# lucidrains/glom-pytorch

Hardware: NVIDIA H100
Metric: column-iterations/sec (BxNxLxiters) at dim=512 L=6 224/14 (higher is better)
Workload: dtype bf16

## Files before the change

### glom_pytorch_b200/csrc/tc_bwd_kernels.cu

```cuda
#include "tc_common.cuh"

#include <stdio.h>

namespace glom {

namespace {

constexpr int BN = 256;
constexpr uint32_t A_BYTES = BM * BK * 2;
constexpr uint32_t B_BYTES = BN * BK * 2;
constexpr uint32_t STAGE_BYTES = A_BYTES + B_BYTES;
constexpr int STAGES = 3;
constexpr int CONSUMER_WARPS = 8;
constexpr int THREADS = 32 * (CONSUMER_WARPS + 1);
constexpr uint32_t PATCH_BYTES = 4096;
constexpr size_t SMEM_BYTES = 1024 + (size_t)STAGES * STAGE_BYTES + 4 * (size_t)STG_BYTES + (size_t)CONSUMER_WARPS * PATCH_BYTES +
                              BN * 4 + 256;

template <int TA, int TB>
__device__ __forceinline__ void kblock(float (&acc)[BN / 2], uint32_t a_smem, uint32_t b_smem) {
  const uint64_t ad = TA ? wgmma_desc_sw128(a_smem, 8192, 1024) : wgmma_desc_sw128(a_smem, 16, 1024);
  const uint64_t bd = TB ? wgmma_desc_sw128(b_smem, 8192, 1024) : wgmma_desc_sw128(b_smem, 16, 1024);
#pragma unroll
  for (int k = 0; k < BK / 16; ++k) wgmma_bf16<BN, TA, TB>(acc, ad + (TA ? (2048 >> 4) : 2) * k, bd + (TB ? (2048 >> 4) : 2) * k);
}

enum { BW_PRE = 0, BW_DH = 1, BW_DX = 2, BW_DW = 3, BW_BATCH = 4 };

struct BwdParams {
  int rows, d, L, n, G;
  int m128;
  int num_tiles;
  const float* b1p;
  __nv_bfloat16* pre;
  __nv_bfloat16* h;
  __nv_bfloat16* dpre;
  float *ds, *d_tokens, *d_pos;
  float *d_bu_w1, *d_bu_w2, *d_td_w1, *d_td_w2;
  float *d_bu_b1, *d_td_b1;
  int bN, bK;
  int a_mn, b_mn;
  int a_state, b_state;
  int out_kind;
  float* out;
  int k_split;
  int a_mn2, b_mn2, a_state2, b_state2;
  const int32_t* steps;
  int t;
  float* dx_td;
  float* b1_part;
  int nbands;
};

__device__ __forceinline__ bool rows_frozen(const BwdParams& p, int r0, int nr, int lane) {
  const int r1 = min(r0 + nr, p.rows);
  bool live = false;
  if (r0 < r1)
    for (int b = r0 / p.n + lane; b <= (r1 - 1) / p.n; b += 32) live |= __ldg(p.steps + b) > p.t;
  return !__any_sync(0xffffffffu, live);
}

__device__ __forceinline__ bool problem_frozen(const BwdParams& p, int z) { return __ldg(p.steps + z / p.L) <= p.t; }

struct Tile {
  int g, m_blk, n_blk, num_kb;
  int kind;
};

template <int MODE>
__device__ __forceinline__ Tile decode(const BwdParams& p, int tile) {
// ... 4 lines not shown
  } else if (MODE == BW_DX) {
    const int nn = p.d / BN, nm = (p.rows + 255) / 256;
    t.n_blk = tile % nn; t.m_blk = (tile / nn) % nm; t.g = tile / (nn * nm); t.num_kb = 4 * p.d / BK;
  } else if (MODE == BW_BATCH) {
    const int nm = (p.n + 255) / 256, nn = (p.bN + BN - 1) / BN;
    t.n_blk = tile % nn; t.m_blk = (tile / nn) % nm; t.g = tile / (nn * nm);
    t.num_kb = p.k_split ? 2 * p.k_split : (p.bK + BK - 1) / BK;
  } else {
    const int per_kind = (p.d / 256) * (4 * p.d / BN);
    t.g = tile / (2 * per_kind);
    const int r = tile % (2 * per_kind);
    t.kind = r / per_kind;
    const int q = r % per_kind;
    const int nn = t.kind == 0 ? 4 * p.d / BN : p.d / BN;
    t.n_blk = q % nn; t.m_blk = q / nn;
    t.num_kb = (p.rows + BK - 1) / BK;
  }
  return t;
}

__device__ __forceinline__ void normal_cdf_pdf(float x, float& cdf, float& pdf) {
  const float a = fabsf(x), t = fminf(a, 6.0f);
  float q = 3.290448512416333e-05f;
  q = fmaf(q, t, -0.0007621519616805017f);
  q = fmaf(q, t, 0.008038812316954136f);
  q = fmaf(q, t, -0.05331535264849663f);
  q = fmaf(q, t, -0.45887142419815063f);
  q = fmaf(q, t, -1.1511567831039429f);
  q = fmaf(q, t, -0.9999995827674866f);
  const float tail = ex2_approx(q);
  cdf = x >= 0.f ? 1.0f - tail : tail;
  float hz = 7.497369551856536e-06f;
  hz = fmaf(hz, t, -0.00023059015802573413f);
  hz = fmaf(hz, t, 0.003048981074243784f);
  hz = fmaf(hz, t, -0.023022783920168877f);
  hz = fmaf(hz, t, 0.11135400831699371f);
  hz = fmaf(hz, t, 0.6360868811607361f);
  hz = fmaf(hz, t, 0.7979033589363098f);
  pdf = tail * hz;
}

template <int MODE, bool DET = false>
__global__ void __launch_bounds__(THREADS, 1)
bwd_gemm_kernel(const __grid_constant__ CUtensorMap map_a0,
                const __grid_constant__ CUtensorMap map_a1,
                const __grid_constant__ CUtensorMap map_a2,
                const __grid_constant__ CUtensorMap map_b,
                const __grid_constant__ CUtensorMap map_b1,
                const __grid_constant__ CUtensorMap map_b2,
                const BwdParams p) {
  extern __shared__ uint8_t smem_raw[];
  uint8_t* smem = smem_raw + ((1024u - (smem_u32(smem_raw) & 1023u)) & 1023u);
  float* stg_all = reinterpret_cast<float*>(smem + (size_t)STAGES * STAGE_BYTES);
  uint8_t* patches = reinterpret_cast<uint8_t*>(stg_all) + 4 * STG_BYTES;
  float* bias_s = reinterpret_cast<float*>(patches + (size_t)CONSUMER_WARPS * PATCH_BYTES);
  uint64_t* full_bar = reinterpret_cast<uint64_t*>(bias_s + BN);
  uint64_t* empty_bar = full_bar + STAGES;

  const int warp = threadIdx.x >> 5, lane = threadIdx.x & 31;
  constexpr int W_TMA = CONSUMER_WARPS;
  const int cta_rank = (int)(blockIdx.x & 1);
  const int cluster_id = blockIdx.x >> 1, num_clusters = gridDim.x >> 1;
  const int kbg_n = 4 * p.d / BK;

  if (warp == W_TMA && lane == 0) {
    for (int i = 0; i < STAGES; ++i) { mbar_init(&full_bar[i], 1); mbar_init(&empty_bar[i], CONSUMER_WARPS); }
    fence_barrier_init();
  }
  __syncthreads();
  pdl_launch_dependents();
  pdl_wait();

  if (warp == W_TMA) {
    const uint32_t elected = elect_one();
    {
      int stage = 0; uint32_t phase = 0;
      for (int tile = cluster_id; tile < p.num_tiles; tile += num_clusters) {
        const Tile t = decode<MODE>(p, tile);
        const int l = t.g >> 1;
        if ((MODE == BW_PRE || MODE == BW_DH || MODE == BW_DX) && p.steps &&
            rows_frozen(p, t.m_blk * 256 + cta_rank * BM, BM, lane))
          continue;
        if (MODE == BW_BATCH && p.steps && problem_frozen(p, t.g)) continue;
        if (MODE == BW_DW && p.steps && rows_frozen(p, 0, p.rows, lane)) continue;
        for (int kb = 0; kb < t.num_kb; ++kb) {
          if (MODE == BW_DW && p.steps && rows_frozen(p, kb * BK, BK, lane)) continue;
          mbar_wait(&empty_bar[stage], phase ^ 1);
          if (elected) {
          const uint32_t sa = smem_u32(smem + (size_t)stage * STAGE_BYTES);
          const uint32_t sb = sa + A_BYTES;
          uint64_t* bar = &full_bar[stage];
          mbar_arrive_expect_tx(bar, STAGE_BYTES);
          if (MODE == BW_PRE || MODE == BW_DH) {
            const int a_row = t.m_blk * 256 + (int)cta_rank * BM;
            const int b_row = t.g * 4 * p.d + t.n_blk * BN;
            if (MODE == BW_PRE) {
              const CUtensorMap* amap = (t.g == 0) ? &map_a0 : ((t.g & 1) ? &map_a2 : &map_a1);
              const int a_col = (t.g == 0) ? 0 : ((t.g & 1) ? l * p.d : (l - 1) * p.d);
              tma_load_2d(sa, amap, bar, a_col + kb * BK, a_row);
            } else {
              tma_load_2d(sa, &map_a0, bar, l * p.d + kb * BK, a_row);
            }
            for (int i = 0; i < 2; ++i) tma_load_2d(sb + i * 16384, &map_b, bar, kb * BK, b_row + i * (BN / 2));
          } else if (MODE == BW_DX) {
            const int m128 = t.m_blk * 2 + (int)cta_rank;
            tma_load_2d(sa, &map_a0, bar, 0, ((t.g * p.m128 + m128) * kbg_n + kb) * BM);
            for (int i = 0; i < 2; ++i) tma_load_2d(sb + i * 16384, &map_b, bar, kb * BK, t.g * p.d + t.n_blk * BN + i * (BN / 2));
          } else if (MODE == BW_BATCH) {
            const int z = t.g, bb = z / p.L, lv = z % p.L;
            const bool seg2 = p.k_split && kb >= p.k_split;
            const int kk = seg2 ? kb - p.k_split : kb;
            const CUtensorMap* am = seg2 ? &map_a1 : &map_a0;
            const CUtensorMap* bm = seg2 ? &map_b1 : &map_b;
            const int a_st = seg2 ? p.a_state2 : p.a_state, b_st = seg2 ? p.b_state2 : p.b_state;
            const int a_mn = seg2 ? p.a_mn2 : p.a_mn, b_mn = seg2 ? p.b_mn2 : p.b_mn;
            const int a_off = a_st ? lv * p.d : 0, a_bt = a_st ? bb : z;
            const int b_off = b_st ? lv * p.d : 0, b_bt = b_st ? bb : z;
            const int mrow = t.m_blk * 256 + cta_rank * BM, ncol = t.n_blk * BN;
            if (!a_mn) tma_load_3d(sa, am, bar, a_off + kk * BK, mrow, a_bt);
            else for (int i = 0; i < 2; ++i) tma_load_3d(sa + i * 8192, am, bar, a_off + mrow + i * 64, kk * BK, a_bt);
            if (!b_mn) for (int i = 0; i < 2; ++i) tma_load_3d(sb + i * 16384, bm, bar, b_off + kk * BK, ncol + i * BM, b_bt);
            else for (int i = 0; i < 4; ++i) tma_load_3d(sb + i * 8192, bm, bar, b_off + ncol + i * 64, kk * BK, b_bt);
          } else {
            const int r0 = kb * BK;
            const int blk_row = (t.g * p.m128 + (r0 >> 7)) * kbg_n;
            const int half = (r0 >> 6) & 1;
            const int mcol = t.m_blk * 256 + cta_rank * BM;
            const int ncol = t.n_blk * BN;
            for (int i = 0; i < 4; ++i) {
              if (t.kind == 0) {
                if (i < 2) tma_load_2d(sa + i * 8192, &map_a0, bar, l * p.d + mcol + i * 64, r0);
                tma_load_2d(sb + i * 8192, &map_a2, bar, 0, (blk_row + (ncol >> 6) + i) * BM + half * 64);
              } else {
                if (i < 2) tma_load_2d(sa + i * 8192, &map_a1, bar, 0, (blk_row + (mcol >> 6) + i) * BM + half * 64);
                const CUtensorMap* bmap = (t.g == 0) ? &map_b : ((t.g & 1) ? &map_b2 : &map_b1);
                const int b_col = (t.g == 0) ? 0 : ((t.g & 1) ? l * p.d : (l - 1) * p.d);
                tma_load_2d(sb + i * 8192, bmap, bar, b_col + ncol + i * 64, r0);
              }
            }
          }
          }
          __syncwarp();
          if (++stage == STAGES) { stage = 0; phase ^= 1; }
        }
      }
    }
  } else if (warp < W_TMA) {
    const int wg = warp >> 2, wi = warp & 3;
    const int quad = warp >> 1, x = warp & 1;
    float* stg = stg_all + quad * (STG_BYTES / 4);
    uint8_t* patch = patches + (size_t)warp * PATCH_BYTES;
    const int c = lane & 7, rsub = lane >> 3;
    const int a_mn1 = (MODE == BW_DW) ? 1 : (MODE == BW_BATCH ? p.a_mn : 0);
    const int b_mn1 = (MODE == BW_DW) ? 1 : (MODE == BW_BATCH ? p.b_mn : 0);
    int stage = 0; uint32_t phase = 0;
    float frag[BN / 2];
    for (int tile = cluster_id; tile < p.num_tiles; tile += num_clusters) {
      const Tile t = decode<MODE>(p, tile);
      if ((MODE == BW_PRE || MODE == BW_DH || MODE == BW_DX) && p.steps &&
          rows_frozen(p, t.m_blk * 256 + cta_rank * BM, BM, lane))
        continue;
      if (MODE == BW_BATCH && p.steps && problem_frozen(p, t.g)) continue;
      if (MODE == BW_DW && p.steps && rows_frozen(p, 0, p.rows, lane)) continue;
      if (MODE == BW_PRE) {
        named_bar_sync(5, CONSUMER_WARPS * 32);
        for (int i = threadIdx.x; i < BN; i += CONSUMER_WARPS * 32) bias_s[i] = __ldg(p.b1p + (size_t)t.g * 4 * p.d + t.n_blk * BN + i);
        named_bar_sync(5, CONSUMER_WARPS * 32);
      }
#pragma unroll
      for (int i = 0; i < BN / 2; ++i) frag[i] = 0.f;
      int prev = -1;
      for (int kb = 0; kb < t.num_kb; ++kb) {
        if (MODE == BW_DW && p.steps && rows_frozen(p, kb * BK, BK, lane)) continue;
        mbar_wait(&full_bar[stage], phase);
        const uint32_t sa = smem_u32(smem + (size_t)stage * STAGE_BYTES) + (uint32_t)wg * 8192u;
        const uint32_t sb = smem_u32(smem + (size_t)stage * STAGE_BYTES) + A_BYTES;
        const bool seg2 = MODE == BW_BATCH && p.k_split && kb >= p.k_split;
        const int sel = seg2 ? 2 * p.a_mn2 + p.b_mn2 : 2 * a_mn1 + b_mn1;
        wgmma_fence_regs(frag);
        wgmma_fence();
        if (sel == 0) kblock<0, 0>(frag, sa, sb);
        else if (sel == 1) kblock<0, 1>(frag, sa, sb);
        else if (sel == 2) kblock<1, 0>(frag, sa, sb);
        else kblock<1, 1>(frag, sa, sb);
        wgmma_commit();
        wgmma_wait<1>();
        wgmma_fence_regs(frag);
        if (prev >= 0) { __syncwarp(); if (lane == 0) mbar_arrive(&empty_bar[prev]); }
        prev = stage;
        if (++stage == STAGES) { stage = 0; phase ^= 1; }
      }
      if (MODE == BW_DW && prev < 0) continue;
      wgmma_wait<0>();
      wgmma_fence_regs(frag);
      __syncwarp();
      if (lane == 0) mbar_arrive(&empty_bar[prev]);
      const int row0 = t.m_blk * 256 + cta_rank * BM + quad * 32;
#pragma unroll 1
      for (int part = 0; part < BN / 64; ++part) {
        const int c0 = 32 * x;
        auto blocked_off = [&](int r) -> size_t {
          const int row = row0 + r, col = t.n_blk * BN + part * 64 + c0 + c * 4;
          return ((size_t)((t.g * p.m128 + (row >> 7)) * kbg_n + (col >> 6)) * BM + (row & 127)) * BK + (col & 63);
        };
        uint2 gp_cur[8];
        if (MODE == BW_DH) {
#pragma unroll
          for (int i = 0; i < 8; ++i) {
            const int r = i * 4 + rsub;
            gp_cur[i] = row0 + r < p.rows ? __ldg(reinterpret_cast<const uint2*>(p.pre + blocked_off(r))) : make_uint2(0u, 0u);
          }
        }
        stage_write(frag, stg, part, wi, lane);
        named_bar_sync(1 + quad, 64);
        uint32_t v[32];
        stage_read(stg, x, lane, v);
#pragma unroll
        for (int j = 0; j < 8; ++j)
          *reinterpret_cast<uint4*>(patch + lane * 128 + ((j ^ (lane & 7)) << 4)) =
              make_uint4(v[4 * j], v[4 * j + 1], v[4 * j + 2], v[4 * j + 3]);
        __syncwarp();
        const int col = t.n_blk * BN + part * 64 + c0 + c * 4;
        float colsum[4] = {0.f, 0.f, 0.f, 0.f};
#pragma unroll
        for (int i = 0; i < 8; ++i) {
          const int r = i * 4 + rsub;
          const float4 acc = *reinterpret_cast<const float4*>(patch + r * 128 + ((c ^ (r & 7)) << 4));
          const int row = row0 + r;
          if (MODE == BW_PRE || MODE == BW_DH) {
            if (row < p.rows) {
              const size_t off = blocked_off(r);
              if (MODE == BW_PRE) {
                const float4 b4 = *reinterpret_cast<const float4*>(bias_s + part * 64 + c0 + c * 4);
                const float xv[4] = {acc.x + b4.x, acc.y + b4.y, acc.z + b4.z, acc.w + b4.w};
                float hv[4], gp[4];
#pragma unroll
                for (int e = 0; e < 4; ++e) {
                  float cdf, pdf;
                  normal_cdf_pdf(xv[e], cdf, pdf);
                  hv[e] = xv[e] * cdf;
                  gp[e] = fmaf(xv[e], pdf, cdf);
                }
                *reinterpret_cast<uint2*>(p.h + off) = make_uint2(pack_bf16x2(hv[0], hv[1]), pack_bf16x2(hv[2], hv[3]));
                *reinterpret_cast<uint2*>(p.pre + off) = make_uint2(pack_bf16x2(gp[0], gp[1]), pack_bf16x2(gp[2], gp[3]));
              } else {
                const uint2 pw = gp_cur[i];
                const float q0 = acc.x * __uint_as_float(pw.x << 16), q1 = acc.y * __uint_as_float(pw.x & 0xFFFF0000u);
                const float q2 = acc.z * __uint_as_float(pw.y << 16), q3 = acc.w * __uint_as_float(pw.y & 0xFFFF0000u);
                colsum[0] += q0; colsum[1] += q1; colsum[2] += q2; colsum[3] += q3;
                *reinterpret_cast<uint2*>(p.dpre + off) = make_uint2(pack_bf16x2(q0, q1), pack_bf16x2(q2, q3));
              }
            }
          } else if (MODE == BW_DX) {
            if constexpr (DET) {
              const int lg = t.g >> 1;
              if (row < p.rows && (t.g & 1)) {
                *reinterpret_cast<float4*>(p.dx_td + ((size_t)row * (p.L - 1) + lg) * p.d + col) = acc;
              } else if (row < p.rows) {
                float* dst = t.g == 0 ? p.d_tokens + (size_t)row * p.d + col : p.ds + ((size_t)row * p.L + lg - 1) * p.d + col;
                float4 o = *reinterpret_cast<const float4*>(dst);
                o.x += acc.x; o.y += acc.y; o.z += acc.z; o.w += acc.w;
                *reinterpret_cast<float4*>(dst) = o;
              }
            } else if (row < p.rows) {
              const int lg = t.g >> 1;
              if (t.g == 0) {
                red_add_f32x4(p.d_tokens + (size_t)row * p.d + col, acc);
              } else if (t.g & 1) {
                red_add_f32x4(p.ds + ((size_t)row * p.L + lg + 1) * p.d + col, acc);
                red_add_f32x4(p.d_pos + (size_t)(row % p.n) * p.d + col, acc);
              } else {
                red_add_f32x4(p.ds + ((size_t)row * p.L + lg - 1) * p.d + col, acc);
              }
            }
          } else if (MODE == BW_BATCH) {
            const int z = t.g;
            if (row < p.n && col < p.bN) {
              if (p.out_kind == 0) {
                float* dst = p.out + ((size_t)z * p.n + row) * p.bN + col;
                if ((p.bN & 3) == 0) *reinterpret_cast<float4*>(dst) = acc;
// ... 166 lines not shown
```

### glom_pytorch_b200/csrc/tc_common.cuh

```cuda
#pragma once
#include "engine.h"
#include "ptx.cuh"

#include <stdio.h>

namespace glom {

constexpr int BM = 128;
constexpr int BK = 64;
constexpr uint32_t A_STAGE_BYTES = BM * BK * 2;

constexpr int STG_PITCH = 68;
constexpr uint32_t STG_BYTES = 32 * STG_PITCH * 4;
template <int S, int R>
__device__ __forceinline__ void stage_write_step(const float (&acc)[R], float* stg, int warp_in_wg, int lane) {
  const int r = 16 * (warp_in_wg & 1) + (lane >> 2), c = 2 * (lane & 3);
#pragma unroll
  for (int j = 0; j < 8; ++j) {
#pragma unroll
    for (int h = 0; h < 2; ++h)
      *reinterpret_cast<float2*>(stg + (r + 8 * h) * STG_PITCH + 8 * j + c) =
          make_float2(acc[4 * (8 * S + j) + 2 * h], acc[4 * (8 * S + j) + 2 * h + 1]);
  }
}
template <int R>
__device__ __forceinline__ void stage_write(const float (&acc)[R], float* stg, int s, int warp_in_wg, int lane) {
  static_assert(R % 32 == 0 && R <= 128, "m64 x N fragment, N in {64, 128, 256}");
  if (s == 0) stage_write_step<0>(acc, stg, warp_in_wg, lane);
  if constexpr (R >= 64) { if (s == 1) stage_write_step<1>(acc, stg, warp_in_wg, lane); }
  if constexpr (R >= 128) {
    if (s == 2) stage_write_step<2>(acc, stg, warp_in_wg, lane);
    if (s == 3) stage_write_step<3>(acc, stg, warp_in_wg, lane);
  }
}
__device__ __forceinline__ void stage_read(const float* stg, int x, int lane, uint32_t (&v)[32]) {
  const float4* src = reinterpret_cast<const float4*>(stg + lane * STG_PITCH + 32 * x);
#pragma unroll
  for (int q = 0; q < 8; ++q) {
    const float4 f = src[q];
    v[4 * q] = __float_as_uint(f.x); v[4 * q + 1] = __float_as_uint(f.y);
    v[4 * q + 2] = __float_as_uint(f.z); v[4 * q + 3] = __float_as_uint(f.w);
  }
}

template <int N, int TB>
__device__ __forceinline__ void wgmma_kblock(float (&acc)[N / 2], uint32_t a_smem, uint32_t b_smem) {
  const uint64_t ad = wgmma_desc_sw128(a_smem, 16, 1024);
  const uint64_t bd = TB ? wgmma_desc_sw128(b_smem, 8192, 1024) : wgmma_desc_sw128(b_smem, 16, 1024);
#pragma unroll
  for (int k = 0; k < BK / 16; ++k) wgmma_bf16<N, 0, TB>(acc, ad + 2 * k, bd + (TB ? (2048 >> 4) : 2) * k);
}

__device__ __forceinline__ float row_chunk_sumsq(float a, float b, float c, float d) {
  float q = a * a;
  q = fmaf(b, b, q);
  q = fmaf(c, c, q);
  q = fmaf(d, d, q);
  q += __shfl_xor_sync(0xffffffffu, q, 1);
  q += __shfl_xor_sync(0xffffffffu, q, 2);
  q += __shfl_xor_sync(0xffffffffu, q, 4);
  return q;
}

struct K2Chunk {
  int l, L, d, n, row0;
  int prow0;
  int s_bcast;
  bool remap;
  const float* s32_in; const __nv_bfloat16* c_in; const float* pos;
  float* s32_out; __nv_bfloat16* sb_out; __nv_bfloat16* sp_out;
};
template <bool FULL, bool SETTLE = false>
__device__ __forceinline__ void k2_chunk(const uint32_t (&v)[32], const float4 b4, uint8_t* patch, const K2Chunk& k,
                                         int col, int lane, int rows_left, float (&rowsq)[8], uint32_t live = ~0u,
                                         float* rowdsq = nullptr, bool want_dsq = false) {
#pragma unroll
  for (int c = 0; c < 8; ++c)
    *reinterpret_cast<uint4*>(patch + lane * 128 + ((c ^ (lane & 7)) << 4)) =
        make_uint4(v[4 * c], v[4 * c + 1], v[4 * c + 2], v[4 * c + 3]);
  __syncwarp();
  const int c = lane & 7, rsub = lane >> 3;
  const bool top = (k.l == k.L - 1);
  const bool has_td = (k.l >= 1);
  const int ld = k.L * k.d, ldp = (k.L - 1) * k.d;
  const size_t base = ((size_t)k.row0 * k.L + k.l) * k.d + col + c * 4;
  const size_t pbase = ((size_t)k.row0 * (k.L - 1) + (k.l - 1)) * k.d + col + c * 4;
#pragma unroll
  for (int h = 0; h < 2; ++h) {
    float4 sv[4], pp[4];
    uint2 cw[4];
#pragma unroll
    for (int j = 0; j < 4; ++j) {
      const int r = (h * 4 + j) * 4 + rsub;
      sv[j] = make_float4(0.f, 0.f, 0.f, 0.f); pp[j] = sv[j]; cw[j] = make_uint2(0u, 0u);
      if ((FULL || r < rows_left) && (!SETTLE || ((live >> r) & 1u))) {
        size_t so = base + (unsigned)(r * ld);
        if (!SETTLE && k.remap) {
          int sr = k.prow0 + r;
          if (k.n >= 32) { if (sr >= k.n) sr -= k.n; } else sr %= k.n;
          so = (size_t)k.l * k.d + col + c * 4 + (unsigned)(sr * ld);
        }
        sv[j] = k.s_bcast ? __ldg(reinterpret_cast<const float4*>(k.s32_in + (size_t)k.l * k.d + col + c * 4))
                          : __ldcs(reinterpret_cast<const float4*>(k.s32_in + so));
        cw[j] = __ldcs(reinterpret_cast<const uint2*>(k.c_in + so));
        if (has_td) {
          int pr = k.prow0 + r;
          if (k.n >= 32) { if (pr >= k.n) pr -= k.n; } else pr %= k.n;
          pp[j] = __ldg(reinterpret_cast<const float4*>(k.pos + (size_t)pr * k.d + col + c * 4));
        }
      }
    }
#pragma unroll
    for (int j = 0; j < 4; ++j) {
      const int i = h * 4 + j;
      const int r = i * 4 + rsub;
      const float4 acc = *reinterpret_cast<const float4*>(patch + r * 128 + ((c ^ (r & 7)) << 4));
      float o0 = (sv[j].x + (acc.x + b4.x)) + __uint_as_float(cw[j].x << 16);
      float o1 = (sv[j].y + (acc.y + b4.y)) + __uint_as_float(cw[j].x & 0xFFFF0000u);
      float o2 = (sv[j].z + (acc.z + b4.z)) + __uint_as_float(cw[j].y << 16);
      float o3 = (sv[j].w + (acc.w + b4.w)) + __uint_as_float(cw[j].y & 0xFFFF0000u);
      if (top) { o0 = o0 / 3.0f; o1 = o1 / 3.0f; o2 = o2 / 3.0f; o3 = o3 / 3.0f; }
      else { o0 *= 0.25f; o1 *= 0.25f; o2 *= 0.25f; o3 *= 0.25f; }
      const bool store = (FULL || r < rows_left) && (!SETTLE || ((live >> r) & 1u));
      if constexpr (SETTLE) if (want_dsq) {
        const float e0 = store ? o0 - sv[j].x : 0.f, e1 = store ? o1 - sv[j].y : 0.f;
        const float e2 = store ? o2 - sv[j].z : 0.f, e3 = store ? o3 - sv[j].w : 0.f;
        rowdsq[i] += row_chunk_sumsq(e0, e1, e2, e3);
      }
      if (store) {
        const size_t o = base + (unsigned)(r * ld);
        __stcs(reinterpret_cast<float4*>(k.s32_out + o), make_float4(o0, o1, o2, o3));
        *reinterpret_cast<uint2*>(k.sb_out + o) = make_uint2(pack_bf16x2(o0, o1), pack_bf16x2(o2, o3));
        if (has_td)
          *reinterpret_cast<uint2*>(k.sp_out + pbase + (unsigned)(r * ldp)) =
              make_uint2(pack_bf16x2(o0 + pp[j].x, o1 + pp[j].y), pack_bf16x2(o2 + pp[j].z, o3 + pp[j].w));
      } else {
        o0 = o1 = o2 = o3 = 0.f;
      }
      rowsq[i] += row_chunk_sumsq(o0, o1, o2, o3);
    }
  }
  __syncwarp();
}

static inline int encode_map(Launch& ln, CUtensorMap* m, const void* base, int rank, const uint64_t* dims,
                             const uint64_t* strides_bytes , const uint32_t* box, const char* what) {
  cuuint64_t gd[3]; cuuint64_t gs[2]; cuuint32_t bx[3]; cuuint32_t es[3] = {1, 1, 1};
  for (int i = 0; i < rank; ++i) { gd[i] = dims[i]; bx[i] = box[i]; }
  for (int i = 0; i < rank - 1; ++i) gs[i] = strides_bytes[i];
  const CUresult r = ln.enc(m, CU_TENSOR_MAP_DATA_TYPE_BFLOAT16, (cuuint32_t)rank, const_cast<void*>(base), gd, gs, bx, es,
                         CU_TENSOR_MAP_INTERLEAVE_NONE, CU_TENSOR_MAP_SWIZZLE_128B, CU_TENSOR_MAP_L2_PROMOTION_L2_256B,
                         CU_TENSOR_MAP_FLOAT_OOB_FILL_NONE);
  if (r != CUDA_SUCCESS) return ln.fail(GLOM_B200_ERR_CUDA, "cuTensorMapEncodeTiled(%s) failed with CUresult %d", what, (int)r);
  return 0;
}

static inline int map2d(Launch& ln, CUtensorMap* m, const void* base, uint64_t rows, uint64_t cols, uint32_t box_rows,
                        const char* what) {
  const uint64_t dims[2] = {cols, rows};
  const uint64_t strides[1] = {cols * 2};
  const uint32_t box[2] = {(uint32_t)BK, box_rows};
  return encode_map(ln, m, base, 2, dims, strides, box, what);
}

}
```

### glom_pytorch_b200/csrc/tc_kernels.cu

```cuda
#include "gemm_sched.cuh"
#include "tc_common.cuh"

#include <stdio.h>
#include <stdlib.h>
#include <string.h>

#include <type_traits>

namespace glom {

constexpr int GEMM_CONSUMER_WARPS = 8;
constexpr int GEMM_THREADS = 128 + 32 * GEMM_CONSUMER_WARPS;
constexpr uint32_t GEMM_PRODUCER_REGS = 40;
constexpr uint32_t GEMM_CONSUMER_REGS = 232;

__device__ unsigned long long g_kernel_clk[PROF_KINDS][8];


template <int MODE, int BN>
struct GemmCfg {
  static constexpr int PARTS = (BN == 256) ? 4 : 2;
  static constexpr int PART_COLS = BN / PARTS;
  static constexpr int THREADS = GEMM_THREADS;
  static constexpr uint32_t B_STAGE_BYTES = BN * BK * 2;
  static constexpr uint32_t STAGE_BYTES = A_STAGE_BYTES + B_STAGE_BYTES;
  static_assert(MODE >= 0 && MODE <= 2, "0 = GEMM1+GELU, 1 = GEMM2+combine, 2 = tokeniser");
  static constexpr int STAGES = (BN == 256) ? 3 : (BN == 128) ? 4 : 5;
  static constexpr uint32_t OUT_BOX_BYTES = 64 * BK * 2;
  static constexpr uint32_t PATCH_BYTES = 4096;
  static constexpr size_t EPI_BYTES = (MODE == 0) ? 2 * (BN / 64) * (size_t)OUT_BOX_BYTES
                                                  : 4 * (size_t)STG_BYTES + (size_t)GEMM_CONSUMER_WARPS * PATCH_BYTES + 4 * 32 * 4;
  static constexpr size_t SMEM_BYTES = 1024  + (size_t)STAGES * STAGE_BYTES + EPI_BYTES + 256 ;
  static_assert(SMEM_BYTES <= 232448, "over the 227 KB of shared memory a block may opt in to");
};

__device__ __forceinline__ void tok_chunk(const uint32_t (&v)[32], const float4 b4, uint8_t* patch, float* dst,
                                          size_t pitch, int lane, int rows_left) {
#pragma unroll
  for (int c = 0; c < 8; ++c)
    *reinterpret_cast<uint4*>(patch + lane * 128 + ((c ^ (lane & 7)) << 4)) =
        make_uint4(v[4 * c], v[4 * c + 1], v[4 * c + 2], v[4 * c + 3]);
  __syncwarp();
  const int c = lane & 7, rsub = lane >> 3;
#pragma unroll
  for (int i = 0; i < 8; ++i) {
    const int r = i * 4 + rsub;
    const float4 a = *reinterpret_cast<const float4*>(patch + r * 128 + ((c ^ (r & 7)) << 4));
    if (r < rows_left)
      *reinterpret_cast<float4*>(dst + (size_t)r * pitch + c * 4) = make_float4(a.x + b4.x, a.y + b4.y, a.z + b4.z, a.w + b4.w);
  }
  __syncwarp();
}

template <int MODE>
__device__ __forceinline__ bool settle_skip(const GemmParams& p, const TileInfo& t) {
  if (p.block_frozen[t.m_blk]) return true;
  return MODE == 0 && t.z == 0 && p.block_fresh != nullptr && !p.block_fresh[t.m_blk];
}

template <int MODE, int BN, bool CNT, bool SETTLE = false>
__global__ void __launch_bounds__(GEMM_THREADS, 1)
gemm_kernel(const __grid_constant__ CUtensorMap map_a0,
            const __grid_constant__ CUtensorMap map_a1,
            const __grid_constant__ CUtensorMap map_a2,
            const __grid_constant__ CUtensorMap map_b,
            const __grid_constant__ CUtensorMap map_out,
            const GemmParams p) {
  using Cfg = GemmCfg<MODE, BN>;
  constexpr int STAGES = Cfg::STAGES;
  constexpr bool RED = MODE != 2 && !SETTLE;
  extern __shared__ uint8_t smem_raw[];
  uint8_t* smem = smem_raw + ((1024u - (smem_u32(smem_raw) & 1023u)) & 1023u);
  uint8_t* epi = smem + (size_t)STAGES * Cfg::STAGE_BYTES;
  float* stg_all = reinterpret_cast<float*>(epi);
  uint8_t* patches = epi + 4 * STG_BYTES;
  float* xch = reinterpret_cast<float*>(patches + (size_t)GEMM_CONSUMER_WARPS * Cfg::PATCH_BYTES);
  uint64_t* full_bar = reinterpret_cast<uint64_t*>(epi + Cfg::EPI_BYTES);
  uint64_t* empty_bar = full_bar + STAGES;

  const int warp = threadIdx.x >> 5;
  const int lane = threadIdx.x & 31;
  constexpr int W_TMA = 0;
  constexpr int W_CONSUMER0 = 4;
  const int cta_rank = (int)(blockIdx.x & 1);
  const int cluster_id = blockIdx.x >> 1;
  const int num_clusters = gridDim.x >> 1;

  if (warp == W_TMA && lane == 0) {
    tma_prefetch_desc(&map_a0);
    tma_prefetch_desc(&map_b);
    if (MODE == 0) { tma_prefetch_desc(&map_a1); tma_prefetch_desc(&map_a2); tma_prefetch_desc(&map_out); }
    for (int i = 0; i < STAGES; ++i) { mbar_init(&full_bar[i], 1); mbar_init(&empty_bar[i], 2 * GEMM_CONSUMER_WARPS); }
    fence_barrier_init();
  }
  cluster_sync_all();
  pdl_launch_dependents();
  pdl_wait();
  const bool clk_thread = blockIdx.x == 0 && warp == W_TMA && lane == 0;
  ClockSample* clk_s = reinterpret_cast<ClockSample*>(empty_bar + STAGES);
  if (clk_thread) *clk_s = clock_sample_begin();
  const bool cnt_cta = CNT && blockIdx.x == 0;
  unsigned long long* const cnt = g_kernel_clk[MODE == 0 ? PROF_GEMM1 : MODE == 1 ? PROF_GEMM2 : PROF_TOKENIZE];
  unsigned long long w0 = 0, w1 = 0;
#define GLOM_CNT_WAIT(acc, stmt) do { if (cnt_cta) { const long long t_ = clock64(); stmt; acc += (unsigned long long)(clock64() - t_); } else { stmt; } } while (0)

  if (warp < W_CONSUMER0) {
    setmaxnreg_dec<GEMM_PRODUCER_REGS>();
    if (warp == W_TMA) {
      const uint32_t elected = elect_one();
      int stage = 0; uint32_t phase = 0;
      const uint32_t smem0 = smem_u32(smem);
      const uint64_t pol_first = l2_policy_evict_first();
      const int kbg_n = 4 * p.d / BK;
      const int blk_skip = (p.m128 - 1) * kbg_n;
      for (int it = 0, tile; (tile = sched_tile<MODE>(p, cluster_id, num_clusters, it)) >= 0; ++it) {
        const TileInfo t = decode_tile<MODE, RED>(p, tile);
        if constexpr (SETTLE) { if (settle_skip<MODE>(p, t)) continue; }
        const CUtensorMap* amap;
        int a_col, b_row;
        if (MODE == 0) {
          const int l = t.z >> 1;
          if (t.z == 0) { amap = &map_a0; a_col = 0; }
          else if (t.z & 1) { amap = &map_a2; a_col = l * p.d; }
          else { amap = &map_a1; a_col = (l - 1) * p.d; }
          b_row = t.z * 4 * p.d + t.n_blk * BN;
        } else if (MODE == 1) {
          amap = &map_a0; a_col = 0;
          b_row = t.z * p.d + t.n_blk * BN;
        } else {
          amap = &map_a0; a_col = 0;
          b_row = t.n_blk * BN;
        }
        const int a_row = t.m_blk * 256 + cta_rank * BM;
        const int blk0 = (2 * t.z * p.m128 + (a_row >> 7)) * kbg_n;
        int td_skip = blk_skip;
        if constexpr (RED && MODE == 1) {
          if (p.num_m_rep > 0 && t.z + 1 >= p.remap_l) td_skip -= ((a_row >> 7) - (a_row >> 7) % p.h_period) * kbg_n;
        }
        for (int kb = 0; kb < t.num_kb; ++kb) {
          GLOM_CNT_WAIT(w0, mbar_wait(&empty_bar[stage], phase ^ 1));
          if (elected) {
            const uint32_t sa = smem0 + (uint32_t)stage * Cfg::STAGE_BYTES;
            uint64_t* bar = &full_bar[stage];
            mbar_arrive_expect_tx(bar, Cfg::STAGE_BYTES);
            if (MODE == 1) {
              const int blk = blk0 + kb + (kb >= kbg_n ? td_skip : 0);
              tma_load_2d_hint(sa, amap, bar, 0, blk * BM, pol_first);
            } else {
              tma_load_2d(sa, amap, bar, a_col + kb * BK, a_row);
            }
            const uint32_t b_half = (uint32_t)cta_rank * (BN / 2);
            tma_load_2d_multicast(sa + A_STAGE_BYTES + b_half * BK * 2, &map_b, bar, kb * BK, b_row + (int)b_half, 0x3);
          }
          __syncwarp();
          if (++stage == STAGES) { stage = 0; phase ^= 1; }
        }
      }
      if (cnt_cta && elected) atomicAdd(&cnt[4], w0);
    }
  } else {
    setmaxnreg_inc<GEMM_CONSUMER_REGS>();
    const int cw = warp - W_CONSUMER0;
    const int wg = cw >> 2, wi = cw & 3;
    const int pair = cw >> 1, x = cw & 1;
    float* stg = stg_all + pair * (STG_BYTES / 4);
    uint8_t* patch = patches + (size_t)cw * Cfg::PATCH_BYTES;
    float* xch_p = xch + pair * 32;
    const uint32_t smem0 = smem_u32(smem);
    const uint64_t pol_stream = l2_policy_evict_first();
    const bool st_issuer = (threadIdx.x & 127) == 0;
    const uint32_t out_wg = smem_u32(epi) + (uint32_t)wg * (BN / 64) * Cfg::OUT_BOX_BYTES;
    const uint32_t st_row = (uint32_t)(16 * wi + 8 * ((lane >> 3) & 1) + (lane & 7)) * 128;
    const int st_jx = lane >> 4, st_sw = lane & 7;
    const uint32_t empty_peer = mapa_shared(smem_u32(empty_bar), (uint32_t)cta_rank ^ 1u);
    auto release = [&](int slot) {
      __syncwarp();
      if (lane == 0) { mbar_arrive(&empty_bar[slot]); mbar_arrive_cluster(empty_peer + 8u * (uint32_t)slot); }
    };
    int stage = 0; uint32_t phase = 0;
    float acc[BN / 2];
    for (int it = 0, tile; (tile = sched_tile<MODE>(p, cluster_id, num_clusters, it)) >= 0; ++it) {
      const TileInfo t = decode_tile<MODE, RED>(p, tile);
      if constexpr (SETTLE) { if (settle_skip<MODE>(p, t)) continue; }
      const int row0 = t.m_blk * 256 + cta_rank * BM + pair * 32;
      const int rows_left = p.rows - row0;
      uint32_t live = ~0u;
      if constexpr (SETTLE && MODE == 1)
        live = __ballot_sync(0xffffffffu, row0 + lane < p.rows && !p.frozen[(row0 + lane) / p.n]);
      bool remap = false;
      if constexpr (RED && MODE == 1) remap = p.num_m_rep > 0 && t.z >= p.remap_l;
      if (MODE == 1 && lane < rows_left) {
        const int src_row = remap ? (row0 + lane) % p.n : row0 + lane;
        const size_t o = ((size_t)src_row * p.L + t.z) * p.d + t.n_blk * BN + x * (BN / 2);
#pragma unroll
        for (int c = 0; c < BN / 2; c += 32) {
          if (!p.s_bcast) prefetch_l2(p.s32_in + o + c);
          if ((c & 63) == 0) prefetch_l2(p.c_in + o + c);
        }
      }
#pragma unroll
      for (int i = 0; i < BN / 2; ++i) acc[i] = 0.f;
      int prev = -1;
      for (int kb = 0; kb < t.num_kb; ++kb) {
        GLOM_CNT_WAIT(w0, mbar_wait(&full_bar[stage], phase));
        const uint32_t sa = smem0 + (uint32_t)stage * Cfg::STAGE_BYTES;
        wgmma_fence_regs(acc);
        wgmma_fence();
        wgmma_kblock<BN, 0>(acc, sa + (uint32_t)wg * (A_STAGE_BYTES / 2), sa + A_STAGE_BYTES);
        wgmma_commit();
        wgmma_wait<1>();
        wgmma_fence_regs(acc);
        if (prev >= 0) release(prev);
        prev = stage;
        if (++stage == STAGES) { stage = 0; phase ^= 1; }
      }
      wgmma_wait<0>();
      wgmma_fence_regs(acc);
      release(prev);
      const long long busy_t0 = cnt_cta ? clock64() : 0;
      if constexpr (MODE == 0) {
        const int wrow0 = t.m_blk * 256 + cta_rank * BM + 64 * wg;
        if (wrow0 < p.rows) {
          const int hblk0 = (t.z * p.m128 + (t.m_blk * 2 + cta_rank)) * (4 * p.d / BK) + t.n_blk * (BN / BK);
          const float* bias = p.bias + (size_t)t.z * 4 * p.d + t.n_blk * BN + 2 * (lane & 3);
          uint32_t pk[BN / 4];
#pragma unroll
          for (int s = 0; s < BN / 64; ++s) {
#pragma unroll
            for (int j = 0; j < 8; ++j) {
              const float2 b = __ldg(reinterpret_cast<const float2*>(bias + 64 * s + 8 * j));
#pragma unroll
              for (int h = 0; h < 2; ++h)
                pk[16 * s + 2 * j + h] = gelu_pair_bf16(acc[4 * (8 * s + j) + 2 * h], acc[4 * (8 * s + j) + 2 * h + 1], b.x, b.y);
            }
          }
          if (st_issuer) bulk_wait_group_read<0>();
          named_bar_sync(1 + wg, 128);
#pragma unroll
          for (int s = 0; s < BN / 64; ++s)
#pragma unroll
            for (int q = 0; q < 4; ++q)
              stmatrix_x4(out_wg + (uint32_t)s * Cfg::OUT_BOX_BYTES + st_row + ((uint32_t)((2 * q + st_jx) ^ st_sw) << 4),
                          pk[16 * s + 4 * q], pk[16 * s + 4 * q + 1], pk[16 * s + 4 * q + 2], pk[16 * s + 4 * q + 3]);
          fence_proxy_async_smem();
          named_bar_sync(1 + wg, 128);
          if (st_issuer) {
#pragma unroll
            for (int s = 0; s < BN / 64; ++s)
              tma_store_2d_hint(&map_out, out_wg + (uint32_t)s * Cfg::OUT_BOX_BYTES, 0, (hblk0 + s) * BM + 64 * wg, pol_stream);
            bulk_commit_group();
          }
        }
      } else {
#pragma unroll 1
        for (int s = 0; s < BN / 64; ++s) {
          stage_write(acc, stg, s, wi, lane);
          named_bar_sync(1 + pair, 64);
          uint32_t v[32];
          stage_read(stg, x, lane, v);
          const int cc = 64 * s + 32 * x;
          if (MODE == 2) {
            float* trow = p.tok_out + (size_t)row0 * p.d + t.n_blk * BN + cc;
            const float4 b4 = __ldg(reinterpret_cast<const float4*>(p.bias + t.n_blk * BN + cc + (lane & 7) * 4));
            tok_chunk(v, b4, patch, trow, (size_t)p.d, lane, rows_left);
          } else {
            K2Chunk kc;
            kc.l = t.z; kc.L = p.L; kc.d = p.d; kc.n = p.n; kc.row0 = row0; kc.prow0 = row0 % p.n; kc.s_bcast = p.s_bcast;
            kc.remap = remap;
            kc.s32_in = p.s32_in; kc.c_in = p.c_in; kc.pos = p.pos;
            kc.s32_out = p.s32_out; kc.sb_out = p.sb_out; kc.sp_out = p.sp_out;
            const int col = t.n_blk * BN + cc;
            const float4 b4 = __ldg(reinterpret_cast<const float4*>(p.bias + (size_t)t.z * p.d + col + (lane & 7) * 4));
            float rowsq[8], rowdsq[8];
#pragma unroll
            for (int i = 0; i < 8; ++i) rowsq[i] = rowdsq[i] = 0.f;
            const bool want_dsq = SETTLE && p.dsq_out != nullptr;
            if (rows_left >= 32) k2_chunk<true, SETTLE>(v, b4, patch, kc, col, lane, 32, rowsq, live, rowdsq, want_dsq);
            else k2_chunk<false, SETTLE>(v, b4, patch, kc, col, lane, rows_left, rowsq, live, rowdsq, want_dsq);
            int part = cc / Cfg::PART_COLS;
            bool writer = true;
            if (Cfg::PART_COLS == 64) {
              float* dxch = reinterpret_cast<float*>(patches + (size_t)(cw | 1) * Cfg::PATCH_BYTES);
              if (x == 1 && (lane & 7) == 0) {
#pragma unroll
                for (int i = 0; i < 8; ++i) xch_p[i * 4 + (lane >> 3)] = rowsq[i];
                if (want_dsq) {
#pragma unroll
                  for (int i = 0; i < 8; ++i) dxch[i * 4 + (lane >> 3)] = rowdsq[i];
                }
              }
              named_bar_sync(1 + pair, 64);
              if (x == 0) {
#pragma unroll
                for (int i = 0; i < 8; ++i) rowsq[i] += xch_p[i * 4 + (lane >> 3)];
                if (want_dsq) {
#pragma unroll
                  for (int i = 0; i < 8; ++i) rowdsq[i] += dxch[i * 4 + (lane >> 3)];
                }
              }
              writer = x == 0;
            }
            if (writer && (lane & 7) == 0) {
              const size_t po = ((size_t)row0 * p.L + t.z) * p.nparts + t.n_blk * Cfg::PARTS + part;
              float* nsq = p.nsq_out + po;
              const int ldn = p.L * p.nparts;
#pragma unroll
              for (int i = 0; i < 8; ++i) {
                const int r = i * 4 + (lane >> 3);
                if (r < rows_left && (!SETTLE || ((live >> r) & 1u))) {
                  nsq[(unsigned)(r * ldn)] = rowsq[i];
                  if (want_dsq) p.dsq_out[po + (unsigned)(r * ldn)] = rowdsq[i];
                }
              }
            }
          }
          named_bar_sync(1 + pair, 64);
        }
      }
      if (cnt_cta) w1 += (unsigned long long)(clock64() - busy_t0);
    }
    if (cnt_cta && cw == 0 && lane == 0) { atomicAdd(&cnt[2], w0); atomicAdd(&cnt[6], w1); }
    if (MODE == 0 && st_issuer) bulk_wait_group<0>();
  }
#undef GLOM_CNT_WAIT

  cluster_sync_all();
  if (clk_thread) clock_sample_end(*clk_s, g_kernel_clk[MODE == 0 ? PROF_GEMM1 : MODE == 1 ? PROF_GEMM2 : PROF_TOKENIZE]);
}

constexpr int ATTN_CONSUMER_WARPS = 8;
constexpr int ATTN_THREADS = 128 + 32 * ATTN_CONSUMER_WARPS;
constexpr uint32_t ATTN_PRODUCER_REGS = 56;
constexpr uint32_t ATTN_CONSUMER_REGS = 224;
constexpr int ATTN_SCALE_WARPS = 3;
constexpr float ATTN_BOUND_MAX = 96.f;
constexpr int ATTN_SINGLE_PASS_MAX = 576;
constexpr int ATTN_PASS_KEYS = 512;

template <int KEYS>
struct AttnCfg {
  static_assert(KEYS == 128 || KEYS == 256, "S block = one wgmma N");
  static constexpr int MAX_KB = (KEYS == 256) ? 1 : 5;
  static constexpr uint32_t SLOT_BYTES = A_STAGE_BYTES + (uint32_t)KEYS * BK * 2;
  static_assert(SLOT_BYTES >= 4 * 8192, "a slot holds a V chunk");
};

struct AttnParams {
  int n, L, d;
  int attend_self, mask_side, mask_d2_max;
  int n_pad16, n_pad64, nkb, nchunk;
// ... 659 lines not shown
```

Before: 67.64 million.

## Read epilogue directly from swizzled staging buffer, drop per-warp patch transpose

The staging buffer now uses an XOR-swizzled 64-float pitch, so epilogue threads can read their row/column float4 straight from it. This removes the extra register round-trip and per-warp patch buffer transpose in the forward and backward epilogues. The freed shared memory goes to deeper TMA pipelines for the non-GELU GEMM modes. k2_chunk also software-pipelines its global loads several rows ahead. The cost is higher register pressure from the prefetch arrays, and the swizzle indexing must match between writer and reader.

```diff
diff --git a/glom_pytorch_b200/csrc/tc_bwd_kernels.cu b/glom_pytorch_b200/csrc/tc_bwd_kernels.cu
--- a/glom_pytorch_b200/csrc/tc_bwd_kernels.cu
+++ b/glom_pytorch_b200/csrc/tc_bwd_kernels.cu
@@ -13,9 +13,7 @@
 constexpr int STAGES = 3;
 constexpr int CONSUMER_WARPS = 8;
 constexpr int THREADS = 32 * (CONSUMER_WARPS + 1);
-constexpr uint32_t PATCH_BYTES = 4096;
-constexpr size_t SMEM_BYTES = 1024 + (size_t)STAGES * STAGE_BYTES + 4 * (size_t)STG_BYTES + (size_t)CONSUMER_WARPS * PATCH_BYTES +
-                              BN * 4 + 256;
+constexpr size_t SMEM_BYTES = 1024 + (size_t)STAGES * STAGE_BYTES + 4 * (size_t)STG_BYTES + BN * 4 + 256;
 
 template <int TA, int TB>
 __device__ __forceinline__ void kblock(float (&acc)[BN / 2], uint32_t a_smem, uint32_t b_smem) {
@@ -126,8 +124,7 @@
   extern __shared__ uint8_t smem_raw[];
   uint8_t* smem = smem_raw + ((1024u - (smem_u32(smem_raw) & 1023u)) & 1023u);
   float* stg_all = reinterpret_cast<float*>(smem + (size_t)STAGES * STAGE_BYTES);
-  uint8_t* patches = reinterpret_cast<uint8_t*>(stg_all) + 4 * STG_BYTES;
-  float* bias_s = reinterpret_cast<float*>(patches + (size_t)CONSUMER_WARPS * PATCH_BYTES);
+  float* bias_s = stg_all + 4 * (STG_BYTES / 4);
   uint64_t* full_bar = reinterpret_cast<uint64_t*>(bias_s + BN);
   uint64_t* empty_bar = full_bar + STAGES;
 
@@ -223,7 +220,6 @@
     const int wg = warp >> 2, wi = warp & 3;
     const int quad = warp >> 1, x = warp & 1;
     float* stg = stg_all + quad * (STG_BYTES / 4);
-    uint8_t* patch = patches + (size_t)warp * PATCH_BYTES;
     const int c = lane & 7, rsub = lane >> 3;
     const int a_mn1 = (MODE == BW_DW) ? 1 : (MODE == BW_BATCH ? p.a_mn : 0);
     const int b_mn1 = (MODE == BW_DW) ? 1 : (MODE == BW_BATCH ? p.b_mn : 0);
@@ -287,19 +283,12 @@
         }
         stage_write(frag, stg, part, wi, lane);
         named_bar_sync(1 + quad, 64);
-        uint32_t v[32];
-        stage_read(stg, x, lane, v);
-#pragma unroll
-        for (int j = 0; j < 8; ++j)
-          *reinterpret_cast<uint4*>(patch + lane * 128 + ((j ^ (lane & 7)) << 4)) =
-              make_uint4(v[4 * j], v[4 * j + 1], v[4 * j + 2], v[4 * j + 3]);
-        __syncwarp();
         const int col = t.n_blk * BN + part * 64 + c0 + c * 4;
         float colsum[4] = {0.f, 0.f, 0.f, 0.f};
 #pragma unroll
         for (int i = 0; i < 8; ++i) {
           const int r = i * 4 + rsub;
-          const float4 acc = *reinterpret_cast<const float4*>(patch + r * 128 + ((c ^ (r & 7)) << 4));
+          const float4 acc = stage_read(stg, x, r, c);
           const int row = row0 + r;
           if (MODE == BW_PRE || MODE == BW_DH) {
             if (row < p.rows) {
diff --git a/glom_pytorch_b200/csrc/tc_common.cuh b/glom_pytorch_b200/csrc/tc_common.cuh
--- a/glom_pytorch_b200/csrc/tc_common.cuh
+++ b/glom_pytorch_b200/csrc/tc_common.cuh
@@ -10,16 +10,18 @@
 constexpr int BK = 64;
 constexpr uint32_t A_STAGE_BYTES = BM * BK * 2;
 
-constexpr int STG_PITCH = 68;
+constexpr int STG_PITCH = 64;
 constexpr uint32_t STG_BYTES = 32 * STG_PITCH * 4;
+__device__ __forceinline__ int stg_swz(int r) { return 2 * (r & 3); }
 template <int S, int R>
 __device__ __forceinline__ void stage_write_step(const float (&acc)[R], float* stg, int warp_in_wg, int lane) {
   const int r = 16 * (warp_in_wg & 1) + (lane >> 2), c = 2 * (lane & 3);
+  const int swz = stg_swz(r);
 #pragma unroll
   for (int j = 0; j < 8; ++j) {
 #pragma unroll
     for (int h = 0; h < 2; ++h)
-      *reinterpret_cast<float2*>(stg + (r + 8 * h) * STG_PITCH + 8 * j + c) =
+      *reinterpret_cast<float2*>(stg + (r + 8 * h) * STG_PITCH + 4 * ((2 * j) ^ swz) + c) =
           make_float2(acc[4 * (8 * S + j) + 2 * h], acc[4 * (8 * S + j) + 2 * h + 1]);
   }
 }
@@ -33,14 +35,8 @@
     if (s == 3) stage_write_step<3>(acc, stg, warp_in_wg, lane);
   }
 }
-__device__ __forceinline__ void stage_read(const float* stg, int x, int lane, uint32_t (&v)[32]) {
-  const float4* src = reinterpret_cast<const float4*>(stg + lane * STG_PITCH + 32 * x);
-#pragma unroll
-  for (int q = 0; q < 8; ++q) {
-    const float4 f = src[q];
-    v[4 * q] = __float_as_uint(f.x); v[4 * q + 1] = __float_as_uint(f.y);
-    v[4 * q + 2] = __float_as_uint(f.z); v[4 * q + 3] = __float_as_uint(f.w);
-  }
+__device__ __forceinline__ float4 stage_read(const float* stg, int x, int r, int c) {
+  return *reinterpret_cast<const float4*>(stg + r * STG_PITCH + 4 * ((8 * x + c) ^ stg_swz(r)));
 }
 
 template <int N, int TB>
@@ -71,76 +67,69 @@
   float* s32_out; __nv_bfloat16* sb_out; __nv_bfloat16* sp_out;
 };
 template <bool FULL, bool SETTLE = false>
-__device__ __forceinline__ void k2_chunk(const uint32_t (&v)[32], const float4 b4, uint8_t* patch, const K2Chunk& k,
-                                         int col, int lane, int rows_left, float (&rowsq)[8], uint32_t live = ~0u,
-                                         float* rowdsq = nullptr, bool want_dsq = false) {
-#pragma unroll
-  for (int c = 0; c < 8; ++c)
-    *reinterpret_cast<uint4*>(patch + lane * 128 + ((c ^ (lane & 7)) << 4)) =
-        make_uint4(v[4 * c], v[4 * c + 1], v[4 * c + 2], v[4 * c + 3]);
-  __syncwarp();
+__device__ __forceinline__ void k2_chunk(const float* stg, int x, const float4 b4, const K2Chunk& k, int col, int lane,
+                                         int rows_left, float (&rowsq)[8], uint32_t live = ~0u, float* rowdsq = nullptr,
+                                         bool want_dsq = false) {
   const int c = lane & 7, rsub = lane >> 3;
   const bool top = (k.l == k.L - 1);
   const bool has_td = (k.l >= 1);
   const int ld = k.L * k.d, ldp = (k.L - 1) * k.d;
   const size_t base = ((size_t)k.row0 * k.L + k.l) * k.d + col + c * 4;
   const size_t pbase = ((size_t)k.row0 * (k.L - 1) + (k.l - 1)) * k.d + col + c * 4;
-#pragma unroll
-  for (int h = 0; h < 2; ++h) {
-    float4 sv[4], pp[4];
-    uint2 cw[4];
-#pragma unroll
-    for (int j = 0; j < 4; ++j) {
-      const int r = (h * 4 + j) * 4 + rsub;
-      sv[j] = make_float4(0.f, 0.f, 0.f, 0.f); pp[j] = sv[j]; cw[j] = make_uint2(0u, 0u);
-      if ((FULL || r < rows_left) && (!SETTLE || ((live >> r) & 1u))) {
-        size_t so = base + (unsigned)(r * ld);
-        if (!SETTLE && k.remap) {
-          int sr = k.prow0 + r;
-          if (k.n >= 32) { if (sr >= k.n) sr -= k.n; } else sr %= k.n;
-          so = (size_t)k.l * k.d + col + c * 4 + (unsigned)(sr * ld);
-        }
-        sv[j] = k.s_bcast ? __ldg(reinterpret_cast<const float4*>(k.s32_in + (size_t)k.l * k.d + col + c * 4))
-                          : __ldcs(reinterpret_cast<const float4*>(k.s32_in + so));
-        cw[j] = __ldcs(reinterpret_cast<const uint2*>(k.c_in + so));
-        if (has_td) {
-          int pr = k.prow0 + r;
-          if (k.n >= 32) { if (pr >= k.n) pr -= k.n; } else pr %= k.n;
-          pp[j] = __ldg(reinterpret_cast<const float4*>(k.pos + (size_t)pr * k.d + col + c * 4));
-        }
+  constexpr int DEPTH = SETTLE ? 4 : 5;
+  float4 sv[8], pp[8];
+  uint2 cw[8];
+  auto load = [&](int i) {
+    const int r = i * 4 + rsub;
+    sv[i] = make_float4(0.f, 0.f, 0.f, 0.f); pp[i] = sv[i]; cw[i] = make_uint2(0u, 0u);
+    if ((FULL || r < rows_left) && (!SETTLE || ((live >> r) & 1u))) {
+      size_t so = base + (unsigned)(r * ld);
+      if (!SETTLE && k.remap) {
+        int sr = k.prow0 + r;
+        if (k.n >= 32) { if (sr >= k.n) sr -= k.n; } else sr %= k.n;
+        so = (size_t)k.l * k.d + col + c * 4 + (unsigned)(sr * ld);
+      }
+      sv[i] = k.s_bcast ? __ldg(reinterpret_cast<const float4*>(k.s32_in + (size_t)k.l * k.d + col + c * 4))
+                        : __ldcs(reinterpret_cast<const float4*>(k.s32_in + so));
+      cw[i] = __ldcs(reinterpret_cast<const uint2*>(k.c_in + so));
+      if (has_td) {
+        int pr = k.prow0 + r;
+        if (k.n >= 32) { if (pr >= k.n) pr -= k.n; } else pr %= k.n;
+        pp[i] = __ldg(reinterpret_cast<const float4*>(k.pos + (size_t)pr * k.d + col + c * 4));
       }
     }
+  };
 #pragma unroll
-    for (int j = 0; j < 4; ++j) {
-      const int i = h * 4 + j;
-      const int r = i * 4 + rsub;
-      const float4 acc = *reinterpret_cast<const float4*>(patch + r * 128 + ((c ^ (r & 7)) << 4));
-      float o0 = (sv[j].x + (acc.x + b4.x)) + __uint_as_float(cw[j].x << 16);
-      float o1 = (sv[j].y + (acc.y + b4.y)) + __uint_as_float(cw[j].x & 0xFFFF0000u);
-      float o2 = (sv[j].z + (acc.z + b4.z)) + __uint_as_float(cw[j].y << 16);
-      float o3 = (sv[j].w + (acc.w + b4.w)) + __uint_as_float(cw[j].y & 0xFFFF0000u);
-      if (top) { o0 = o0 / 3.0f; o1 = o1 / 3.0f; o2 = o2 / 3.0f; o3 = o3 / 3.0f; }
-      else { o0 *= 0.25f; o1 *= 0.25f; o2 *= 0.25f; o3 *= 0.25f; }
-      const bool store = (FULL || r < rows_left) && (!SETTLE || ((live >> r) & 1u));
-      if constexpr (SETTLE) if (want_dsq) {
-        const float e0 = store ? o0 - sv[j].x : 0.f, e1 = store ? o1 - sv[j].y : 0.f;
-        const float e2 = store ? o2 - sv[j].z : 0.f, e3 = store ? o3 - sv[j].w : 0.f;
-        rowdsq[i] += row_chunk_sumsq(e0, e1, e2, e3);
-      }
-      if (store) {
-        const size_t o = base + (unsigned)(r * ld);
-        __stcs(reinterpret_cast<float4*>(k.s32_out + o), make_float4(o0, o1, o2, o3));
-        *reinterpret_cast<uint2*>(k.sb_out + o) = make_uint2(pack_bf16x2(o0, o1), pack_bf16x2(o2, o3));
-        if (has_td)
-          *reinterpret_cast<uint2*>(k.sp_out + pbase + (unsigned)(r * ldp)) =
-              make_uint2(pack_bf16x2(o0 + pp[j].x, o1 + pp[j].y), pack_bf16x2(o2 + pp[j].z, o3 + pp[j].w));
-      } else {
-        o0 = o1 = o2 = o3 = 0.f;
-      }
-      rowsq[i] += row_chunk_sumsq(o0, o1, o2, o3);
+  for (int i = 0; i < DEPTH; ++i) load(i);
+#pragma unroll
+  for (int i = 0; i < 8; ++i) {
+    const int r = i * 4 + rsub;
+    const float4 acc = stage_read(stg, x, r, c);
+    float o0 = (sv[i].x + (acc.x + b4.x)) + __uint_as_float(cw[i].x << 16);
+    float o1 = (sv[i].y + (acc.y + b4.y)) + __uint_as_float(cw[i].x & 0xFFFF0000u);
+    float o2 = (sv[i].z + (acc.z + b4.z)) + __uint_as_float(cw[i].y << 16);
+    float o3 = (sv[i].w + (acc.w + b4.w)) + __uint_as_float(cw[i].y & 0xFFFF0000u);
+    if (top) { o0 = o0 / 3.0f; o1 = o1 / 3.0f; o2 = o2 / 3.0f; o3 = o3 / 3.0f; }
+    else { o0 *= 0.25f; o1 *= 0.25f; o2 *= 0.25f; o3 *= 0.25f; }
+    const bool store = (FULL || r < rows_left) && (!SETTLE || ((live >> r) & 1u));
+    if constexpr (SETTLE) if (want_dsq) {
+      const float e0 = store ? o0 - sv[i].x : 0.f, e1 = store ? o1 - sv[i].y : 0.f;
+      const float e2 = store ? o2 - sv[i].z : 0.f, e3 = store ? o3 - sv[i].w : 0.f;
+      rowdsq[i] += row_chunk_sumsq(e0, e1, e2, e3);
     }
+    if (store) {
+      const size_t o = base + (unsigned)(r * ld);
+      __stcs(reinterpret_cast<float4*>(k.s32_out + o), make_float4(o0, o1, o2, o3));
+      *reinterpret_cast<uint2*>(k.sb_out + o) = make_uint2(pack_bf16x2(o0, o1), pack_bf16x2(o2, o3));
+      if (has_td)
+        *reinterpret_cast<uint2*>(k.sp_out + pbase + (unsigned)(r * ldp)) =
+            make_uint2(pack_bf16x2(o0 + pp[i].x, o1 + pp[i].y), pack_bf16x2(o2 + pp[i].z, o3 + pp[i].w));
+    } else {
+      o0 = o1 = o2 = o3 = 0.f;
+    }
+    rowsq[i] += row_chunk_sumsq(o0, o1, o2, o3);
+    if (i + DEPTH < 8) load(i + DEPTH);
   }
-  __syncwarp();
 }
 
 static inline int encode_map(Launch& ln, CUtensorMap* m, const void* base, int rank, const uint64_t* dims,
diff --git a/glom_pytorch_b200/csrc/tc_kernels.cu b/glom_pytorch_b200/csrc/tc_kernels.cu
--- a/glom_pytorch_b200/csrc/tc_kernels.cu
+++ b/glom_pytorch_b200/csrc/tc_kernels.cu
@@ -25,31 +25,25 @@
   static constexpr uint32_t B_STAGE_BYTES = BN * BK * 2;
   static constexpr uint32_t STAGE_BYTES = A_STAGE_BYTES + B_STAGE_BYTES;
   static_assert(MODE >= 0 && MODE <= 2, "0 = GEMM1+GELU, 1 = GEMM2+combine, 2 = tokeniser");
-  static constexpr int STAGES = (BN == 256) ? 3 : (BN == 128) ? 4 : 5;
+  static constexpr int STAGES = (MODE == 0) ? ((BN == 256) ? 3 : (BN == 128) ? 4 : 5)
+                                            : ((BN == 256) ? 4 : (BN == 128) ? 6 : 8);
   static constexpr uint32_t OUT_BOX_BYTES = 64 * BK * 2;
-  static constexpr uint32_t PATCH_BYTES = 4096;
   static constexpr size_t EPI_BYTES = (MODE == 0) ? 2 * (BN / 64) * (size_t)OUT_BOX_BYTES
-                                                  : 4 * (size_t)STG_BYTES + (size_t)GEMM_CONSUMER_WARPS * PATCH_BYTES + 4 * 32 * 4;
+                                                  : 4 * (size_t)STG_BYTES + 2 * 4 * 32 * 4;
   static constexpr size_t SMEM_BYTES = 1024  + (size_t)STAGES * STAGE_BYTES + EPI_BYTES + 256 ;
   static_assert(SMEM_BYTES <= 232448, "over the 227 KB of shared memory a block may opt in to");
 };
 
-__device__ __forceinline__ void tok_chunk(const uint32_t (&v)[32], const float4 b4, uint8_t* patch, float* dst,
-                                          size_t pitch, int lane, int rows_left) {
-#pragma unroll
-  for (int c = 0; c < 8; ++c)
-    *reinterpret_cast<uint4*>(patch + lane * 128 + ((c ^ (lane & 7)) << 4)) =
-        make_uint4(v[4 * c], v[4 * c + 1], v[4 * c + 2], v[4 * c + 3]);
-  __syncwarp();
+__device__ __forceinline__ void tok_chunk(const float* stg, int x, const float4 b4, float* dst, size_t pitch, int lane,
+                                          int rows_left) {
   const int c = lane & 7, rsub = lane >> 3;
 #pragma unroll
   for (int i = 0; i < 8; ++i) {
     const int r = i * 4 + rsub;
-    const float4 a = *reinterpret_cast<const float4*>(patch + r * 128 + ((c ^ (r & 7)) << 4));
+    const float4 a = stage_read(stg, x, r, c);
     if (r < rows_left)
       *reinterpret_cast<float4*>(dst + (size_t)r * pitch + c * 4) = make_float4(a.x + b4.x, a.y + b4.y, a.z + b4.z, a.w + b4.w);
   }
-  __syncwarp();
 }
 
 template <int MODE>
@@ -73,8 +67,8 @@
   uint8_t* smem = smem_raw + ((1024u - (smem_u32(smem_raw) & 1023u)) & 1023u);
   uint8_t* epi = smem + (size_t)STAGES * Cfg::STAGE_BYTES;
   float* stg_all = reinterpret_cast<float*>(epi);
-  uint8_t* patches = epi + 4 * STG_BYTES;
-  float* xch = reinterpret_cast<float*>(patches + (size_t)GEMM_CONSUMER_WARPS * Cfg::PATCH_BYTES);
+  float* xch = stg_all + 4 * (STG_BYTES / 4);
+  float* dxch = xch + 4 * 32;
   uint64_t* full_bar = reinterpret_cast<uint64_t*>(epi + Cfg::EPI_BYTES);
   uint64_t* empty_bar = full_bar + STAGES;
 
@@ -164,8 +158,8 @@
     const int wg = cw >> 2, wi = cw & 3;
     const int pair = cw >> 1, x = cw & 1;
     float* stg = stg_all + pair * (STG_BYTES / 4);
-    uint8_t* patch = patches + (size_t)cw * Cfg::PATCH_BYTES;
     float* xch_p = xch + pair * 32;
+    float* dxch_p = dxch + pair * 32;
     const uint32_t smem0 = smem_u32(smem);
     const uint64_t pol_stream = l2_policy_evict_first();
     const bool st_issuer = (threadIdx.x & 127) == 0;
@@ -256,13 +250,11 @@
         for (int s = 0; s < BN / 64; ++s) {
           stage_write(acc, stg, s, wi, lane);
           named_bar_sync(1 + pair, 64);
-          uint32_t v[32];
-          stage_read(stg, x, lane, v);
           const int cc = 64 * s + 32 * x;
           if (MODE == 2) {
             float* trow = p.tok_out + (size_t)row0 * p.d + t.n_blk * BN + cc;
             const float4 b4 = __ldg(reinterpret_cast<const float4*>(p.bias + t.n_blk * BN + cc + (lane & 7) * 4));
-            tok_chunk(v, b4, patch, trow, (size_t)p.d, lane, rows_left);
+            tok_chunk(stg, x, b4, trow, (size_t)p.d, lane, rows_left);
           } else {
             K2Chunk kc;
             kc.l = t.z; kc.L = p.L; kc.d = p.d; kc.n = p.n; kc.row0 = row0; kc.prow0 = row0 % p.n; kc.s_bcast = p.s_bcast;
@@ -275,18 +267,17 @@
 #pragma unroll
             for (int i = 0; i < 8; ++i) rowsq[i] = rowdsq[i] = 0.f;
             const bool want_dsq = SETTLE && p.dsq_out != nullptr;
-            if (rows_left >= 32) k2_chunk<true, SETTLE>(v, b4, patch, kc, col, lane, 32, rowsq, live, rowdsq, want_dsq);
-            else k2_chunk<false, SETTLE>(v, b4, patch, kc, col, lane, rows_left, rowsq, live, rowdsq, want_dsq);
+            if (rows_left >= 32) k2_chunk<true, SETTLE>(stg, x, b4, kc, col, lane, 32, rowsq, live, rowdsq, want_dsq);
+            else k2_chunk<false, SETTLE>(stg, x, b4, kc, col, lane, rows_left, rowsq, live, rowdsq, want_dsq);
             int part = cc / Cfg::PART_COLS;
             bool writer = true;
             if (Cfg::PART_COLS == 64) {
-              float* dxch = reinterpret_cast<float*>(patches + (size_t)(cw | 1) * Cfg::PATCH_BYTES);
               if (x == 1 && (lane & 7) == 0) {
 #pragma unroll
                 for (int i = 0; i < 8; ++i) xch_p[i * 4 + (lane >> 3)] = rowsq[i];
                 if (want_dsq) {
 #pragma unroll
-                  for (int i = 0; i < 8; ++i) dxch[i * 4 + (lane >> 3)] = rowdsq[i];
+                  for (int i = 0; i < 8; ++i) dxch_p[i * 4 + (lane >> 3)] = rowdsq[i];
                 }
               }
               named_bar_sync(1 + pair, 64);
@@ -295,7 +286,7 @@
                 for (int i = 0; i < 8; ++i) rowsq[i] += xch_p[i * 4 + (lane >> 3)];
                 if (want_dsq) {
 #pragma unroll
-                  for (int i = 0; i < 8; ++i) rowdsq[i] += dxch[i * 4 + (lane >> 3)];
+                  for (int i = 0; i < 8; ++i) rowdsq[i] += dxch_p[i * 4 + (lane >> 3)];
                 }
               }
               writer = x == 0;
```

Result: faster. 69.17 million, median of 6 (+2.3%).
